# nianticlabs/relpose-gnn

Measured on AMD Instinct MI355X. Metric: graphs/sec (8-node fully-connected, 224x224), higher is better.
Workload: dtype f32; 1 GPU; BASELINE.json configs[1]: batch=32 8-node fully-connected graphs per GPU, 224x224 RGB, fp32, ResNet34 + GNN (D=2048, gnn_recursion=2, droprate=0, eval), random-init weights; nodes_per_graph=8, edges_per_graph=56, streams_per_gpu=2, loaded_library=relpose-gnn_amd/lib/librelpose_gnn_hip.so@88d037e48742

## Files before the change

relpose-gnn_amd/csrc/stem.hip:

```cpp
#include "rpg_common.h"

typedef float f32x16 __attribute__((ext_vector_type(16)));

namespace {

constexpr int ST_NT = 512;
constexpr int PH = 4;
constexpr int CR = 2 * PH + 1;
constexpr int IR = 2 * CR + 5;
constexpr int TWP_MAX = 56;
constexpr int PITCH = 4 * TWP_MAX + 8;
constexpr int KP = 74;
constexpr int NF = 2;
constexpr int NFRAG_MAX = (CR * (2 * TWP_MAX + 1) + 31) / 32;
constexpr int PATCH_FLOATS = 3 * IR * PITCH;
constexpr int POOL_FLOATS = (PH * TWP_MAX + 1) * 64;
constexpr int TAB_DWORDS = NFRAG_MAX * 32 * 4;
constexpr int ST_LDS_BYTES = (PATCH_FLOATS + POOL_FLOATS + TAB_DWORDS) * 4;

struct StemArgs {
    const float* x;
    const float* wpack;
    const float* shift;
    float* out;
    int N, H, W, Hc, Wc, Hp, Wp;
    int TWp, tiles_x, tiles_y, RW, nfrag, total_tiles;
    int nbx, nblk, ncl;
};

__host__ __device__ constexpr int tap_off(int c, int kh, int kw) { return (c * IR + kh) * PITCH + kw; }
__host__ __device__ constexpr int pair_class(int kp) { return kp < 63 ? 0 : (kp < 72 ? 1 : (kp == 72 ? 2 : 0)); }
__host__ __device__ constexpr int pair_off(int kp) {
    return kp < 63 ? tap_off(kp / 21, (kp % 21) / 3, 2 * (kp % 3))
                   : (kp < 72 ? tap_off((kp - 63) / 3, 2 * ((kp - 63) % 3), 6) : (kp == 72 ? tap_off(0, 6, 6) : tap_off(2, 6, 6)));
}

__global__ __launch_bounds__(ST_NT) void stem_pool_kernel(StemArgs a) {
    extern __shared__ __attribute__((aligned(16))) float lds[];
    float* patch = lds;
    unsigned* pooled = reinterpret_cast<unsigned*>(lds + PATCH_FLOATS);
    uint4* tab = reinterpret_cast<uint4*>(lds + PATCH_FLOATS + POOL_FLOATS);
    const int tid = threadIdx.x, lane = tid & 63, h = lane >> 5;
    const int wave = __builtin_amdgcn_readfirstlane(tid >> 6);

    float breg[KP][NF];
#pragma unroll
    for (int kp = 0; kp < KP; ++kp)
#pragma unroll
        for (int nf = 0; nf < NF; ++nf) breg[kp][nf] = a.wpack[(kp * NF + nf) * 64 + lane];
    float sh[NF];
#pragma unroll
    for (int nf = 0; nf < NF; ++nf) sh[nf] = a.shift[32 * nf + (lane & 31)];
    __builtin_amdgcn_s_waitcnt(0x0F70);
#pragma unroll
    for (int kp = 0; kp < KP; ++kp)
#pragma unroll
        for (int nf = 0; nf < NF; ++nf) asm volatile("" : "+v"(breg[kp][nf]));
#pragma unroll
    for (int nf = 0; nf < NF; ++nf) asm volatile("" : "+v"(sh[nf]));
    const unsigned trash = (unsigned)(PH * a.TWp) * 256u;
    const unsigned lane_b = 4u * (unsigned)(lane & 31);
    const int pcol = tid & 255, prow0 = __builtin_amdgcn_readfirstlane(tid >> 8);
    constexpr int NROW = 3 * IR, NPV = (NROW + 1) / 2;
    for (int tile = blockIdx.x; tile < a.total_tiles; tile += gridDim.x) {
        const int n = tile / (a.tiles_y * a.tiles_x);
        const int tr = tile - n * (a.tiles_y * a.tiles_x);
        const int ty = tr / a.tiles_x, tx = tr - ty * a.tiles_x;
        const int P0 = ty * PH, Q0 = tx * a.TWp;
        const int cy0 = 2 * P0 - 1, cx0 = 2 * Q0 - 1;
        const int iy0 = 2 * cy0 - 3, ix0 = 2 * cx0 - 3;
        const int npix = CR * a.RW;
        {
            float pv[NPV];
            {
                const float* img = a.x + (size_t)n * 3 * a.H * a.W;
                const int ix = ix0 + pcol;
                const int ixc = ix < 0 ? 0 : (ix >= a.W ? a.W - 1 : ix);
#pragma unroll
                for (int u = 0; u < NPV; ++u) {
                    int rr = prow0 + 2 * u;
                    rr = rr < NROW ? rr : NROW - 1;
                    const int c = rr / IR, r = rr - c * IR;
                    int iy = iy0 + r;
                    iy = iy < 0 ? 0 : (iy >= a.H ? a.H - 1 : iy);
#ifndef ST_NO_PATCH
                    pv[u] = img[((size_t)c * a.H + iy) * a.W + ixc];
#else
                    pv[u] = 1.f;
#endif
                }
            }
            for (int i = tid; i < (PH * a.TWp + 1) * 16; i += ST_NT) reinterpret_cast<uint4*>(pooled)[i] = make_uint4(0u, 0u, 0u, 0u);
            for (int l = tid; l < (a.nfrag - a.nblk) * 32; l += ST_NT) {
                int ey = CR - 1, ex = l;
                bool in = l < a.RW;
                if (!in && a.ncl > 0) {
                    const int l2 = l - a.RW;
                    ey = l2 / a.ncl;
                    ex = 8 * a.nbx + (l2 - ey * a.ncl);
                    in = ey < CR - 1;
                }
                const int cy = cy0 + ey, cx = cx0 + ex;
                unsigned c4[4] = {trash, trash, trash, trash};
                if (in && (unsigned)cy < (unsigned)a.Hc && (unsigned)cx < (unsigned)a.Wc) {
                    const int r0 = (cy >> 1) - P0, r1 = ((cy + 1) >> 1) - P0, q0 = (cx >> 1) - Q0, q1 = ((cx + 1) >> 1) - Q0;
                    const bool r0v = (unsigned)r0 < (unsigned)PH && P0 + r0 < a.Hp, r1v = r1 != r0 && (unsigned)r1 < (unsigned)PH && P0 + r1 < a.Hp;
                    const bool q0v = (unsigned)q0 < (unsigned)a.TWp && Q0 + q0 < a.Wp, q1v = q1 != q0 && (unsigned)q1 < (unsigned)a.TWp && Q0 + q1 < a.Wp;
                    if (r0v && q0v) c4[0] = (unsigned)(r0 * a.TWp + q0) * 256u;
                    if (r0v && q1v) c4[1] = (unsigned)(r0 * a.TWp + q1) * 256u;
                    if (r1v && q0v) c4[2] = (unsigned)(r1 * a.TWp + q0) * 256u;
                    if (r1v && q1v) c4[3] = (unsigned)(r1 * a.TWp + q1) * 256u;
                }
                tab[l] = make_uint4(c4[0], c4[1], c4[2], c4[3]);
            }
            if (pcol < PITCH) {
                const bool col_ok = pcol < 4 * a.TWp + 7 && (unsigned)(ix0 + pcol) < (unsigned)a.W;
#pragma unroll
                for (int u = 0; u < NPV; ++u) {
                    const int rr = prow0 + 2 * u;
                    const int r = rr - (rr / IR) * IR;
                    const bool ok = col_ok && (unsigned)(iy0 + r) < (unsigned)a.H;
                    if (rr < NROW) patch[rr * PITCH + pcol] = ok ? pv[u] : 0.f;
                }
            }
        }
        __syncthreads();
        for (int f = wave; f < a.nfrag; f += ST_NT / 64) {
            const bool blk = f < a.nblk;
            int oy, ox, by = 0, bx = 0;
            if (blk) {
                by = f / a.nbx; bx = f - by * a.nbx;
                oy = 4 * by + ((lane & 31) >> 3);
                ox = 8 * bx + (lane & 7);
            } else {
                const int l = (f - a.nblk) * 32 + (lane & 31);
                oy = CR - 1; ox = l;
                if (l >= a.RW) {
                    const int l2 = l - a.RW;
                    oy = a.ncl > 0 ? l2 / a.ncl : CR;
                    ox = 8 * a.nbx + (l2 - oy * a.ncl);
                    if (oy >= CR - 1) { oy = 0; ox = 0; }
                }
            }
            const float* q = patch + (2 * oy * PITCH + 2 * ox);
            const float* q0 = q + (h ? 1 : 0);
            const float* q1 = q + (h ? PITCH : 0);
            const float* q2 = q + (h ? IR * PITCH : 0);
            f32x16 acc[NF];
#pragma unroll
            for (int nf = 0; nf < NF; ++nf)
#pragma unroll
                for (int e = 0; e < 16; ++e) acc[nf][e] = 0.f;
#pragma unroll
            for (int kp = 0; kp < KP; ++kp) {
                const int cls = pair_class(kp);
                const float av = (cls == 0 ? q0 : (cls == 1 ? q1 : q2))[pair_off(kp)];
#pragma unroll
                for (int nf = 0; nf < NF; ++nf) {
#ifndef ST_NO_MFMA
                    acc[nf] = __builtin_amdgcn_mfma_f32_32x32x2f32(av, breg[kp][nf], acc[nf], 0, 0, 0);
#else
                    acc[nf][kp & 15] += av * breg[kp][nf];
#endif
                }
            }
#ifdef ST_NO_EPI
            if (a.N == -5)
#endif
            if (blk) {
                const int cyb = cy0 + 4 * by, cxs = cx0 + 8 * bx + 4 * h;
                bool rok[4], cok[4];
#pragma unroll
                for (int t = 0; t < 4; ++t) {
                    rok[t] = (unsigned)(cyb + t) < (unsigned)a.Hc;
                    cok[t] = (unsigned)(cxs + t) < (unsigned)a.Wc;
                }
                const int ra = 2 * by, qa = 4 * bx + 2 * h;
                unsigned cell[3][3];
#pragma unroll
                for (int ri = 0; ri < 3; ++ri)
#pragma unroll
                    for (int qi = 0; qi < 3; ++qi) {
                        const int r = ra - 1 + ri, qq = qa - 1 + qi;
                        const bool ok = (unsigned)r < (unsigned)PH && P0 + r < a.Hp && (unsigned)qq < (unsigned)a.TWp && Q0 + qq < a.Wp;
                        cell[ri][qi] = (ok ? (unsigned)(r * a.TWp + qq) * 256u : trash) + lane_b;
                    }
#pragma unroll
                for (int nf = 0; nf < NF; ++nf) {
                    float c[4][3];
#pragma unroll
                    for (int y = 0; y < 4; ++y) {
                        float v[4];
#pragma unroll
                        for (int xx = 0; xx < 4; ++xx) {
                            const float t = rpg::relu(acc[nf][4 * y + xx] + sh[nf]);
                            v[xx] = rok[y] && cok[xx] ? t : 0.f;
                        }
                        c[y][0] = v[0];
                        c[y][1] = rpg::nan_max3(v[0], v[1], v[2]);
                        c[y][2] = rpg::nan_max(v[2], v[3]);
                    }
#pragma unroll
                    for (int qi = 0; qi < 3; ++qi) {
                        const float m0 = c[0][qi];
                        const float m1 = rpg::nan_max3(c[0][qi], c[1][qi], c[2][qi]);
                        const float m2 = rpg::nan_max(c[2][qi], c[3][qi]);
                        const float m[3] = {m0, m1, m2};
#pragma unroll
                        for (int ri = 0; ri < 3; ++ri) {
                            if ((ri == 0 || qi == 0) && __builtin_amdgcn_ballot_w64(cell[ri][qi] != trash + lane_b) == 0) continue;
#ifndef ST_NO_ATOMICS
                            atomicMax(reinterpret_cast<unsigned*>(reinterpret_cast<char*>(pooled) + cell[ri][qi]) + 32 * nf,
                                      __float_as_uint(m[ri]));
#else
                            asm volatile("" ::"v"(cell[ri][qi]), "v"(m[ri]));
#endif
                        }
                    }
                }
            } else {
                const int l0 = (f - a.nblk) * 32 + 4 * h;
#pragma unroll
                for (int e = 0; e < 16; ++e) {
                    const uint4 cells = tab[l0 + (e & 3) + 8 * (e >> 2)];
                    const unsigned v0 = __float_as_uint(rpg::relu(acc[0][e] + sh[0]));
                    const unsigned v1 = __float_as_uint(rpg::relu(acc[1][e] + sh[1]));
                    const unsigned co[4] = {cells.x, cells.y, cells.z, cells.w};
#pragma unroll
                    for (int k = 0; k < 4; ++k) {
                        if (k > 0 && __builtin_amdgcn_ballot_w64(co[k] != trash) == 0) continue;
                        unsigned* cellp = reinterpret_cast<unsigned*>(reinterpret_cast<char*>(pooled) + (co[k] + lane_b));
#ifndef ST_NO_ATOMICS
                        atomicMax(cellp, v0);
                        atomicMax(cellp + 32, v1);
#else
                        asm volatile("" ::"v"(cellp), "v"(v0), "v"(v1));
#endif
                    }
                }
            }
        }
        __syncthreads();
        for (int i = tid; i < PH * a.TWp * 16; i += ST_NT) {
            const int c4 = i & 15, cell = i >> 4;
            const int r = cell / a.TWp, qq = cell - r * a.TWp;
            const int py = P0 + r, px = Q0 + qq;
            if (py < a.Hp && px < a.Wp)
                reinterpret_cast<uint4*>(a.out)[(((size_t)n * a.Hp + py) * a.Wp + px) * 16 + c4] = reinterpret_cast<const uint4*>(pooled)[i];
        }
        __syncthreads();
    }
}


constexpr int SF_NT = 256, SF_TP = 15, SF_NW = 75;
struct StemSFArgs {
    const float* x;
    const float* wpack;
    const float* shift;
    float* out;
    int N, H, W, Hc, Wc, Hp, Wp;
    int TP, tiles_x, BH, bands;
    unsigned items;
};

__global__ __launch_bounds__(SF_NT) __attribute__((amdgpu_waves_per_eu(2, 2))) void stem_strip_f32_kernel(StemSFArgs a) {
    constexpr int NFH = 1;
    constexpr unsigned SENT = 0x80000000u;
    __shared__ float wl[2 * SF_NW * 64];
    __shared__ __attribute__((aligned(16))) float shl[64];
    const int tid = threadIdx.x, lane = tid & 63, l = lane & 31, h = lane >> 5;
    const int wave = __builtin_amdgcn_readfirstlane(tid >> 6);
    for (int i = tid; i < 2 * SF_NW * 64; i += SF_NT) wl[i] = a.wpack[i];
    if (tid < 64) shl[tid] = a.shift[tid];
    __syncthreads();
    const unsigned b = blockIdx.x, nb = gridDim.x;
    unsigned wg = b;
    if ((nb & 15u) == 0) { const unsigned xcd = b & 7u, k = b >> 3; wg = ((k >> 1) * 8u + xcd) * 2u + (k & 1u); }
    const unsigned item = wg * 4u + (unsigned)wave;
    if (item >= a.items) return;
    const int nf = NFH == 1 ? (int)(item & 1u) : 0;
    unsigned rest = NFH == 1 ? item >> 1 : item;
    const int strip = (int)(rest % (unsigned)a.tiles_x); rest /= (unsigned)a.tiles_x;
    const int band = (int)(rest % (unsigned)a.bands);
    const int n = (int)(rest / (unsigned)a.bands);
    const int Q0 = strip * a.TP, P0 = band * a.BH;
    const int nq = a.TP < a.Wp - Q0 ? a.TP : a.Wp - Q0, np = a.BH < a.Hp - P0 ? a.BH : a.Hp - P0;
    const int H = a.H, W = a.W;
    const bool hi = h != 0;

    const int u = l < 16 ? 2 * l : 2 * (l - 16) + 1;
    int cx = 2 * Q0 - 1 + u;
    cx = cx < 0 ? 0 : (cx >= a.Wc ? a.Wc - 1 : cx);
    unsigned vcol[4];
#pragma unroll
    for (int q = 0; q < 4; ++q) {
        const int col = q < 3 ? 2 * cx - 3 + 2 * q + h : 2 * cx + 3;
        vcol[q] = (unsigned)col < (unsigned)W ? 4u * (unsigned)col : SENT;
    }
    const size_t img_elems = (size_t)3 * H * W;
    const __amdgpu_buffer_rsrc_t rs =
        __builtin_amdgcn_make_buffer_rsrc(const_cast<float*>(a.x) + (size_t)n * img_elems, 0, (unsigned)(img_elems * 4), 0x00020000);

    float win[3][8][4];
#pragma unroll
    for (int c = 0; c < 3; ++c)
#pragma unroll
        for (int sl = 0; sl < 8; ++sl)
#pragma unroll
            for (int q = 0; q < 4; ++q) win[c][sl][q] = 0.f;
    float mx[NFH][16];
    const float* const wl_lane = wl + nf * SF_NW * 64 + lane;
    float* const out_n = a.out + (size_t)n * a.Hp * a.Wp * 64 + 32 * nf + 4 * h;
    auto emit = [&](int py) {
        if (py < P0 || py >= P0 + np) return;
#pragma unroll
        for (int f = 0; f < NFH; ++f) {
            float r[16];
#pragma unroll
            for (int e = 0; e < 16; ++e) {
                const int mi = __builtin_bit_cast(int, mx[f][e]);
                const float right = __builtin_bit_cast(float, __builtin_amdgcn_update_dpp(mi, mi, 0x101, 0xf, 0xf, false));
                const float odd = __builtin_bit_cast(float, __builtin_amdgcn_ds_swizzle(mi, 0x401f));
                r[e] = rpg::nan_max3(mx[f][e], right, odd);
            }
            if (l < nq) {
                float* o = out_n + ((size_t)py * a.Wp + Q0 + l) * 64 + 32 * f;
#pragma unroll
                for (int g = 0; g < 4; ++g) {
                    const float4 sh = *reinterpret_cast<const float4*>(shl + 32 * (nf + f) + 8 * g + 4 * h);
                    float4 v;
                    v.x = rpg::relu(r[4 * g + 0] + sh.x); v.y = rpg::relu(r[4 * g + 1] + sh.y);
                    v.z = rpg::relu(r[4 * g + 2] + sh.z); v.w = rpg::relu(r[4 * g + 3] + sh.w);
                    *reinterpret_cast<float4*>(o + 8 * g) = v;
                }
            }
        }
    };

    const int oy_first = P0 > 0 ? 2 * P0 - 1 : 0;
    int oy_last = 2 * (P0 + np) - 1;
    oy_last = oy_last < a.Hc ? oy_last : a.Hc - 1;
#define RPG_SF_LOAD(SL, ROW)                                                                                                   \
    do {                                                                                                                       \
        const int r_ = (ROW);                                                                                                  \
        if ((unsigned)r_ < (unsigned)H) {                                                                                      \
            _Pragma("unroll") for (int c = 0; c < 3; ++c) {                                                                    \
                const unsigned ro_ = (unsigned)(((c * H + r_) * W) * 4);                                                       \
                _Pragma("unroll") for (int q = 0; q < 4; ++q)                                                                  \
                    win[c][SL][q] = __builtin_bit_cast(float, __builtin_amdgcn_raw_buffer_load_b32(rs, vcol[q] == SENT ? SENT : vcol[q] + ro_, 0, 0)); \
            }                                                                                                                  \
        } else {                                                                                                               \
            _Pragma("unroll") for (int c = 0; c < 3; ++c)                                                                      \
                _Pragma("unroll") for (int q = 0; q < 4; ++q) win[c][SL][q] = 0.f;                                             \
        }                                                                                                                      \
    } while (0)
#define RPG_SF_MFMA(K, B)                                                                                                      \
    do {                                                                                                                       \
        _Pragma("unroll") for (int f = 0; f < NFH; ++f) {                                                                      \
            acc[f] = __builtin_amdgcn_mfma_f32_32x32x2f32(wf[f][(K) % 3], (B), acc[f], 0, 0, 0);                               \
            if ((K) + 2 < SF_NW) wf[f][((K) + 2) % 3] = wl_lane[(f * SF_NW + (K) + 2) * 64];                                   \
            __builtin_amdgcn_sched_barrier(0);                                                                                 \
        }                                                                                                                      \
    } while (0)
#define RPG_SF_ROW(R)                                                                                                          \
    do {                                                                                                                       \
        RPG_SF_LOAD((2 * (R) + 3) & 7, 2 * oy + 3);                                  \
        RPG_SF_LOAD((2 * (R) + 4) & 7, 2 * oy + 4);                                          \
        if (oy >= oy_first) {                                                                                                  \
            f32x16 acc[NFH];         \
            float wf[NFH][3];                                                                                                  \
            _Pragma("unroll") for (int f = 0; f < NFH; ++f) {                                                                  \
                _Pragma("unroll") for (int e = 0; e < 16; ++e) acc[f][e] = 0.f;                                                \
                wf[f][0] = wl_lane[(f * SF_NW + 0) * 64];                                                                      \
                wf[f][1] = wl_lane[(f * SF_NW + 1) * 64];                                                                      \
            }                                                                                                                  \
            __builtin_amdgcn_sched_barrier(0);                                                                                 \
            _Pragma("unroll") for (int kh = 0; kh < 7; ++kh) {                                                                 \
                const int sl_ = (2 * (R) + 5 + kh) & 7, kb_ = 9 * kh + 3 * (kh / 2);                                           \
                _Pragma("unroll") for (int c = 0; c < 3; ++c)                                                                  \
                    _Pragma("unroll") for (int p = 0; p < 3; ++p) RPG_SF_MFMA(kb_ + 3 * c + p, win[c][sl_][p]);                \
                if (kh & 1) {                                                                                                  \
                    _Pragma("unroll") for (int c = 0; c < 3; ++c)                                                              \
                        RPG_SF_MFMA(kb_ + 9 + c, hi ? win[c][sl_][3] : win[c][(sl_ + 7) & 7][3]);                              \
                }                                                                                                              \
                if (kh == 6) {                                                                                                 \
                    _Pragma("unroll") for (int c = 0; c < 3; ++c) RPG_SF_MFMA(kb_ + 9 + c, win[c][sl_][3]);                    \
                }                                                                                                              \
            }                                                                                                                  \
            if (oy == oy_first) {                                                                                              \
                _Pragma("unroll") for (int f = 0; f < NFH; ++f)                                                                \
                    _Pragma("unroll") for (int e = 0; e < 16; ++e) mx[f][e] = acc[f][e];                                    \
            } else {                                                                                                           \
                _Pragma("unroll") for (int f = 0; f < NFH; ++f)                                                                \
                    _Pragma("unroll") for (int e = 0; e < 16; ++e) mx[f][e] = rpg::nan_max(mx[f][e], acc[f][e]);           \
            }                                                                                                                  \
            if ((R) & 1) {                                                                                                     \
                emit((oy - 1) >> 1);                                                                                           \
                _Pragma("unroll") for (int f = 0; f < NFH; ++f)                                                                \
                    _Pragma("unroll") for (int e = 0; e < 16; ++e) mx[f][e] = acc[f][e];                                    \
            }                                                                                                                  \
        }                                                                                                                      \
        ++oy;                                                                                                                  \
    } while (0)

    int oy = (oy_first - 3) & ~3;
    while (oy <= oy_last) {
        RPG_SF_ROW(0);
        if (oy > oy_last) break;
        RPG_SF_ROW(1);
        if (oy > oy_last) break;
        RPG_SF_ROW(2);
        if (oy > oy_last) break;
        RPG_SF_ROW(3);
    }
#undef RPG_SF_ROW
#undef RPG_SF_MFMA
#undef RPG_SF_LOAD
    if (!(oy_last & 1)) emit(oy_last >> 1);
}

}

namespace rpg {

bool stem_pool_supported(int h, int w, int cout) { return tuning().stem.fused && cout == 64 && h >= 1 && w >= 1; }


static int strip_band_rows(long items_per_band, int hp, long slots) {
    int best_bh = hp;
    double best = -1.0;
    for (int bands = 1; bands <= hp; ++bands) {
        const int bh = (hp + bands - 1) / bands;
        if (bh < 7 && bands > 1) break;
        const int nb = (hp + bh - 1) / bh;
        if (nb != bands) continue;
        const long wgs = (items_per_band * nb + 3) / 4;
        const long rounds = (wgs + slots - 1) / slots;
        const double eff = (double)wgs / (double)(rounds * slots) * (2.0 * bh / (2.0 * bh + 2.5)) * ((double)hp / (double)(nb * bh));
        if (eff > best + 1e-9) { best = eff; best_bh = bh; }
    }
    return best_bh;
}

int launch_stem_pool(const float* x_nchw, const float* wpack, const float* shift, float* out, int n, int h, int w,
                     hipStream_t s) {
    if (!x_nchw || !wpack || !shift || !out || n <= 0 || h <= 0 || w <= 0 || !aligned16(out)) return RPG_ERR_BAD_ARG;
    if (tuning().stem.strip && (long)3 * h * w * 4 < (1L << 31)) {
        StemSFArgs sa{};
        sa.x = x_nchw; sa.wpack = wpack + KP * NF * 64; sa.shift = shift; sa.out = out;
        sa.N = n; sa.H = h; sa.W = w;
        sa.Hc = (h + 6 - 7) / 2 + 1; sa.Wc = (w + 6 - 7) / 2 + 1;
        sa.Hp = (sa.Hc + 2 - 3) / 2 + 1; sa.Wp = (sa.Wc + 2 - 3) / 2 + 1;
        sa.tiles_x = (sa.Wp + SF_TP - 1) / SF_TP;
        sa.TP = (sa.Wp + sa.tiles_x - 1) / sa.tiles_x;
        if (tuning().stem.strip_bh > 0) {
            sa.BH = tuning().stem.strip_bh < sa.Hp ? tuning().stem.strip_bh : sa.Hp;
        } else {
            sa.BH = strip_band_rows((long)n * sa.tiles_x * 2, sa.Hp, 2L * num_cus());
        }
        sa.bands = (sa.Hp + sa.BH - 1) / sa.BH;
        const long items = (long)n * sa.bands * sa.tiles_x * 2;
        if (items + 64 < (1L << 32)) {
            sa.items = (unsigned)items;
            const int slot = timing_begin(RPG_TIMER_CONV, s);
            hipLaunchKernelGGL(stem_strip_f32_kernel, dim3((unsigned)((items + 3) / 4)), dim3(SF_NT), 0, s, sa);
            timing_end(slot, 2.0 * (double)n * sa.Hc * sa.Wc * 64.0 * 147.0, s,
                       (double)items * (2.0 * sa.Hp / sa.bands + 1.0) * SF_NW * 4096.0);
            RPG_CHECK_LAUNCH("stem_conv_bn_relu_maxpool (strips)");
            return RPG_OK;
        }
    }
    StemArgs a{};
    a.x = x_nchw; a.wpack = wpack; a.shift = shift; a.out = out;
    a.N = n; a.H = h; a.W = w;
    a.Hc = (h + 6 - 7) / 2 + 1; a.Wc = (w + 6 - 7) / 2 + 1;
    a.Hp = (a.Hc + 2 - 3) / 2 + 1; a.Wp = (a.Wc + 2 - 3) / 2 + 1;
    a.tiles_x = (a.Wp + TWP_MAX - 1) / TWP_MAX;
    a.TWp = (a.Wp + a.tiles_x - 1) / a.tiles_x;
    a.tiles_y = (a.Hp + PH - 1) / PH;
    a.RW = 2 * a.TWp + 1;
    a.nbx = a.RW / 8;
    a.nblk = 2 * a.nbx;
    a.ncl = a.RW - 8 * a.nbx;
    a.nfrag = a.nblk + (a.RW + 8 * a.ncl + 31) / 32;
    const long total = (long)n * a.tiles_y * a.tiles_x;
    if (total >= (1L << 31) || (long)n * 3 * h * w >= (1L << 40)) return RPG_ERR_BAD_ARG;
    a.total_tiles = (int)total;
    int dev = 0;
    if (hipGetDevice(&dev) != hipSuccess || dev < 0 || dev >= 64) dev = 0;
    static bool attr[64] = {};
    if (!attr[dev]) {
        (void)hipFuncSetAttribute(reinterpret_cast<const void*>(stem_pool_kernel), hipFuncAttributeMaxDynamicSharedMemorySize,
                                  ST_LDS_BYTES);
        attr[dev] = true;
    }
    const int slot = timing_begin(RPG_TIMER_CONV, s);
    const int grid = (int)(total < num_cus() ? total : num_cus());
    hipLaunchKernelGGL(stem_pool_kernel, dim3(grid), dim3(ST_NT), ST_LDS_BYTES, s, a);
    timing_end(slot, 2.0 * (double)n * a.Hc * a.Wc * 64.0 * 147.0, s, (double)total * a.nfrag * KP * NF * 4096.0);
    RPG_CHECK_LAUNCH("stem_conv_bn_relu_maxpool");
    return RPG_OK;
}

}

extern "C" int rpg_stem_conv7x7s2_bn_relu_maxpool_f32(const float* x_nchw, const float* wpack, const float* shift,
                                                      float* y_nhwc, int n, int h, int w, void* stream) {
    return rpg::launch_stem_pool(x_nchw, wpack, shift, y_nhwc, n, h, w, rpg::as_stream(stream));
}

extern "C" int rpg_stem_pair_table(int* tap_a , int* tap_b ) {
    if (!tap_a || !tap_b) return RPG_ERR_BAD_ARG;
    for (int kp = 0; kp < KP; ++kp) {
        const int off = pair_off(kp);
        const int c = off / (IR * PITCH), kh = (off / PITCH) % IR, kw = off % PITCH;
        tap_a[3 * kp] = c; tap_a[3 * kp + 1] = kh; tap_a[3 * kp + 2] = kw;
        const int cls = pair_class(kp);
        int cb = c + (cls == 2), khb = kh + (cls == 1), kwb = kw + (cls == 0);
        if (cb > 2 || khb > 6 || kwb > 6) cb = -1;
        tap_b[3 * kp] = cb; tap_b[3 * kp + 1] = khb; tap_b[3 * kp + 2] = kwb;
    }
    return RPG_OK;
}
```

relpose-gnn_amd/csrc/tuning.h:

```cpp
#pragma once
#include "../../include/relpose_gnn_hip.h"

namespace rpg {

struct Tuning {
    struct Gemm {
        int force_tile;
        int bk;
        int epi_lds, streamk;
        int fast;
        int waves8;
        int sk_min_its;
        int fold_k;
        int lin112;
        int inkernel_fixup;
        int fixup_prio;
    } gemm;
    struct Gnn {
        int split, fuse_agg;
        int mean_first;
    } gnn;
    struct Wino {
        int on;
        int min_blocks;
        int split;
        int split_steps;
        int persist;
        int combine_max;
        int wino2d;
    } wino;
    struct Bf16 {
        int bk, fast, tile, dma, linear_dma, lean_epi, pair, persist, tail;
        int patch, stages;
        int chunk, chunk_mb;
        int fuse_block;
        int ws64;
        int fused_stem;
        int stem_strip;
        int stem_strip_bh;
    } bf16;
    struct Stem {
        int fused;
        int strip, strip_bh;
    } stem;
};

struct TuningRow {
    int key;
    const char* name;
    int def;
    bool (*valid)(int);
    void (*decode)(Tuning&, int);
};

constexpr int kTuningKeys = 32;

#define RPG_TUNING_ROW(NAME, def, valid, decode) \
    {RPG_TUNE_##NAME, #NAME, def, [](int v) -> bool { (void)v; return valid; }, [](Tuning& t, int v) { (void)t; (void)v; decode; }}

inline constexpr TuningRow kTuningRows[kTuningKeys] = {
    RPG_TUNING_ROW(TILE, -1, true, t.gemm.force_tile = v),
    RPG_TUNING_ROW(BK, 0, v == 0 || v == 16 || v == 32, t.gemm.bk = v),
    RPG_TUNING_ROW(EPILOGUE, 1, true, t.gemm.epi_lds = v != 0),
    RPG_TUNING_ROW(STREAMK, 1, true, t.gemm.streamk = v != 0),
    RPG_TUNING_ROW(WINOGRAD, 1, v >= 0 && !(v > 3 && v < 16),
                   if (v >= 16) { t.wino.on = 1; t.wino.min_blocks = v; } else { t.wino.on = v; t.wino.min_blocks = 16; }),
    RPG_TUNING_ROW(GNN_SPLIT, 1, true, t.gnn.split = v != 0),
    RPG_TUNING_ROW(BF16_BK, 32, v == 32 || v == 64, t.bf16.bk = v),
    RPG_TUNING_ROW(FAST_LOADER, 1, true, t.gemm.fast = v != 0),
    RPG_TUNING_ROW(WINO_SPLIT, 1, v >= 0 && v <= 96,
                   t.wino.split = v != 0; t.wino.split_steps = v >= 2 ? v : 3),
    RPG_TUNING_ROW(BF16_FAST, 1, true, t.bf16.fast = v != 0),
    RPG_TUNING_ROW(FUSED_STEM, 1, true,
                   t.stem.fused = (v & 1) != 0; t.stem.strip = (v & 128) != 0; t.stem.strip_bh = (v >> 8) > 0 ? (v >> 8) : 0;
                   t.bf16.fused_stem = (v & 1) != 0; t.bf16.stem_strip = (v & 2) ? 0 : ((v & 32) ? 1 : 9);
                   t.bf16.stem_strip_bh = (v >> 8) > 0 ? (v >> 8) : 0),
    RPG_TUNING_ROW(WAVES8, 1, true, t.gemm.waves8 = v != 0),
    RPG_TUNING_ROW(WINO_SHORT, 0, v >= 0, ),
    RPG_TUNING_ROW(GNN_FUSE_AGG, 1, true,
                   t.gnn.fuse_agg = v != 0; t.gnn.mean_first = v != 0 && v != 2),
    RPG_TUNING_ROW(WINO_PERSIST, 1, v >= 0 && v <= 2, t.wino.persist = v),
    RPG_TUNING_ROW(BF16_TILE, -1, v >= -1 && v <= 3, t.bf16.tile = v),
    RPG_TUNING_ROW(BF16_DMA, 1, v >= 0 && v <= 40, t.bf16.dma = v),
    RPG_TUNING_ROW(BF16_PATCH, 1, v >= 0 && v % 10 <= 4 && v <= 14,
                   t.bf16.stages = v >= 10 ? 3 : 4; t.bf16.patch = v % 10),
#ifdef RPG_PROBE_WS64
    RPG_TUNING_ROW(BF16_WS64, 0, v >= 0 && v <= 2, t.bf16.ws64 = v),
#else
    RPG_TUNING_ROW(BF16_WS64, 0, v == 0, t.bf16.ws64 = v),
#endif
    RPG_TUNING_ROW(SK_MIN_ITS, 8, v >= 1 && v <= 4096, t.gemm.sk_min_its = v),
    RPG_TUNING_ROW(INKERNEL_FIXUP, 0, v >= 0 && v <= 7,
                   t.gemm.inkernel_fixup = v & 3; t.wino.combine_max = (v & 4) ? 32 : 8),
    RPG_TUNING_ROW(BF16_CHUNK, 0, v >= 0,
                   t.bf16.chunk = v & 4095; t.bf16.chunk_mb = (v >> 12) ? (v >> 12) : 64),
#ifdef RPG_PROBE_WINO2D
    RPG_TUNING_ROW(WINO2D, 0, v >= 0 && v <= 2, t.wino.wino2d = v),
#else
    RPG_TUNING_ROW(WINO2D, 0, v == 0, t.wino.wino2d = v),
#endif
    RPG_TUNING_ROW(BF16_LEAN_EPI, 1, true, t.bf16.lean_epi = v != 0),
    RPG_TUNING_ROW(BF16_LINEAR_DMA, 0, v == 0 || (v >= 10 && v <= 19), t.bf16.linear_dma = v),
    RPG_TUNING_ROW(BF16_PERSIST, 0, true, t.bf16.persist = v != 0),
    RPG_TUNING_ROW(FOLD_K, 256, v >= 0 && v % 64 == 0, t.gemm.fold_k = v),
    RPG_TUNING_ROW(BF16_FUSE_BLOCK, 3, true, t.bf16.fuse_block = v & 7),
    RPG_TUNING_ROW(BF16_TAIL, 1, v >= 0 && v <= 7, t.bf16.tail = v & 7),
    RPG_TUNING_ROW(LIN112, 3, v >= 0 && v <= 3, t.gemm.lin112 = v),
    RPG_TUNING_ROW(FIXUP_PRIO, 0, true, t.gemm.fixup_prio = v != 0),
    RPG_TUNING_ROW(BF16_PAIR, 1, true, t.bf16.pair = v != 0),
};
#undef RPG_TUNING_ROW

constexpr bool tuning_rows_in_key_order() {
    for (int k = 0; k < kTuningKeys; ++k)
        if (kTuningRows[k].key != k) return false;
    return true;
}
static_assert(tuning_rows_in_key_order(), "kTuningRows[k] must be the row of key k");

struct TuningState {
    int raw[kTuningKeys];
    Tuning decoded;
};

constexpr TuningState default_tuning_state() {
    TuningState s{};
    for (int k = 0; k < kTuningKeys; ++k) {
        s.raw[k] = kTuningRows[k].def;
        kTuningRows[k].decode(s.decoded, s.raw[k]);
    }
    return s;
}

inline TuningState g_tuning_state = default_tuning_state();

inline const Tuning& tuning() { return g_tuning_state.decoded; }

inline const TuningRow* tuning_row(int key) { return key >= 0 && key < kTuningKeys ? &kTuningRows[key] : nullptr; }

inline int set_tuning(int key, int value) {
    const TuningRow* row = tuning_row(key);
    if (!row || !row->valid(value)) return RPG_ERR_BAD_ARG;
    g_tuning_state.raw[key] = value;
    row->decode(g_tuning_state.decoded, value);
    return RPG_OK;
}

inline int get_tuning(int key, int* value, int* default_value) {
    const TuningRow* row = tuning_row(key);
    if (!row) return RPG_ERR_BAD_ARG;
    if (value) *value = g_tuning_state.raw[key];
    if (default_value) *default_value = row->def;
    return RPG_OK;
}

}
```

Before: 3186 graphs/s.

## Add exact-strip fp32 stem conv+pool kernel and make it the default path

Adds a new strip kernel for the fused 7x7 stem conv + BN + ReLU + maxpool. Each wave keeps a sliding register window of input rows loaded through buffer loads, with out-of-range rows and columns masked via a sentinel offset. It runs one chain of MFMA 32x32x2 f32 over the exact filter taps per conv row, with weights staged in LDS. With default tuning (strip bit off, tile bit off), this kernel now replaces the previous tiled stem path. The goal is to cut redundant input staging and LDS traffic in the stem, at the cost of more register pressure and extra per-lane gather loads.

Result: no change. 3212 graphs/s (median of 6 runs) (+0.8%).

```diff
diff --git a/relpose-gnn_amd/csrc/stem.hip b/relpose-gnn_amd/csrc/stem.hip
--- a/relpose-gnn_amd/csrc/stem.hip
+++ b/relpose-gnn_amd/csrc/stem.hip
@@ -420,6 +420,166 @@
     if (!(oy_last & 1)) emit(oy_last >> 1);
 }
 
+__device__ __forceinline__ float pick(bool second, float b, float a) { return second ? b : a; }
+
+__global__ __launch_bounds__(SF_NT) __attribute__((amdgpu_waves_per_eu(2, 2))) void stem_strip_exact_kernel(StemSFArgs a) {
+    constexpr unsigned SENT = 0x80000000u;
+    __shared__ float wl[KP * NF * 64];
+    __shared__ __attribute__((aligned(16))) float shl[64];
+    const int tid = threadIdx.x, lane = tid & 63, l = lane & 31, h = lane >> 5;
+    const int wave = __builtin_amdgcn_readfirstlane(tid >> 6);
+    for (int i = tid; i < KP * NF * 64; i += SF_NT) wl[i] = a.wpack[i];
+    if (tid < 64) shl[tid] = a.shift[tid];
+    __syncthreads();
+    const unsigned b = blockIdx.x, nb = gridDim.x;
+    unsigned wg = b;
+    if ((nb & 15u) == 0) { const unsigned xcd = b & 7u, k = b >> 3; wg = ((k >> 1) * 8u + xcd) * 2u + (k & 1u); }
+    const unsigned item = wg * 4u + (unsigned)wave;
+    if (item >= a.items) return;
+    const int nf = (int)(item & 1u);
+    unsigned rest = item >> 1;
+    const int strip = (int)(rest % (unsigned)a.tiles_x); rest /= (unsigned)a.tiles_x;
+    const int band = (int)(rest % (unsigned)a.bands);
+    const int n = (int)(rest / (unsigned)a.bands);
+    const int Q0 = strip * a.TP, P0 = band * a.BH;
+    const int nq = a.TP < a.Wp - Q0 ? a.TP : a.Wp - Q0, np = a.BH < a.Hp - P0 ? a.BH : a.Hp - P0;
+    const int H = a.H, W = a.W;
+    const bool hi = h != 0;
+
+    const int u = l < 16 ? 2 * l : 2 * (l - 16) + 1;
+    int cx = 2 * Q0 - 1 + u;
+    cx = cx < 0 ? 0 : (cx >= a.Wc ? a.Wc - 1 : cx);
+    unsigned vcol[5];
+#pragma unroll
+    for (int q = 0; q < 5; ++q) {
+        const int col = q < 3 ? 2 * cx - 3 + 2 * q + h : (q == 3 ? 2 * cx + 3 : 2 * cx + 3 + h);
+        vcol[q] = (unsigned)col < (unsigned)W ? 4u * (unsigned)col : SENT;
+    }
+    const size_t img_elems = (size_t)3 * H * W;
+    const __amdgpu_buffer_rsrc_t rs =
+        __builtin_amdgcn_make_buffer_rsrc(const_cast<float*>(a.x) + (size_t)n * img_elems, 0, (unsigned)(img_elems * 4), 0x00020000);
+
+    float win[3][8][4];
+#pragma unroll
+    for (int c = 0; c < 3; ++c)
+#pragma unroll
+        for (int sl = 0; sl < 8; ++sl)
+#pragma unroll
+            for (int q = 0; q < 4; ++q) win[c][sl][q] = 0.f;
+    float mx[16];
+    const float* const wl_lane = wl + nf * 64 + lane;
+    float* const out_n = a.out + (size_t)n * a.Hp * a.Wp * 64 + 32 * nf + 4 * h;
+    auto emit = [&](int py) {
+        if (py < P0 || py >= P0 + np) return;
+        float r[16];
+#pragma unroll
+        for (int e = 0; e < 16; ++e) {
+            const int mi = __builtin_bit_cast(int, mx[e]);
+            const float right = __builtin_bit_cast(float, __builtin_amdgcn_update_dpp(mi, mi, 0x101, 0xf, 0xf, false));
+            const float odd = __builtin_bit_cast(float, __builtin_amdgcn_ds_swizzle(mi, 0x401f));
+            r[e] = rpg::nan_max3(mx[e], right, odd);
+        }
+        if (l < nq) {
+            float* o = out_n + ((size_t)py * a.Wp + Q0 + l) * 64;
+#pragma unroll
+            for (int g = 0; g < 4; ++g) {
+                const float4 sh = *reinterpret_cast<const float4*>(shl + 32 * nf + 8 * g + 4 * h);
+                float4 v;
+                v.x = rpg::relu(r[4 * g + 0] + sh.x); v.y = rpg::relu(r[4 * g + 1] + sh.y);
+                v.z = rpg::relu(r[4 * g + 2] + sh.z); v.w = rpg::relu(r[4 * g + 3] + sh.w);
+                *reinterpret_cast<float4*>(o + 8 * g) = v;
+            }
+        }
+    };
+
+    const int oy_first = P0 > 0 ? 2 * P0 - 1 : 0;
+    int oy_last = 2 * (P0 + np) - 1;
+    oy_last = oy_last < a.Hc ? oy_last : a.Hc - 1;
+    const int row_min = 2 * oy_first - 3 > 0 ? 2 * oy_first - 3 : 0;
+    const unsigned row_cnt = (unsigned)(H - row_min);
+#define RPG_SX_SLOT(R, KH) ((2 * (R) + 5 + (KH)) & 7)
+#define RPG_SX_LOAD(C, SL, ROW, EVEN)                                                                                          \
+    do {                                                                                                                       \
+        const int r_ = (ROW);                                                                                                  \
+        const bool rok_ = (unsigned)(r_ - row_min) < row_cnt;        \
+        unsigned ro_ = (unsigned)((((C) * H + r_) * W) * 4);                                                                   \
+        asm volatile("" : "+s"(ro_));         \
+        _Pragma("unroll") for (int q = 0; q < 4; ++q) {                                                                        \
+            const unsigned vc_ = vcol[(q == 3 && (C) == 2 && (EVEN)) ? 4 : q];                                                 \
+            win[C][SL][q] = __builtin_bit_cast(float, __builtin_amdgcn_raw_buffer_load_b32(rs, rok_ && vc_ != SENT ? vc_ + ro_ : SENT, 0, 0)); \
+        }                                                                                                                      \
+    } while (0)
+#define RPG_SX_MFMA(K, B)                                                                                                      \
+    do {                                                                                                                       \
+        acc = __builtin_amdgcn_mfma_f32_32x32x2f32(wf[(K) % 3], (B), acc, 0, 0, 0);                                            \
+        if ((K) + 2 < KP) wf[((K) + 2) % 3] = wl_lane[((K) + 2) * (NF * 64)];                                                  \
+        __builtin_amdgcn_sched_barrier(0);                                                                                     \
+    } while (0)
+#define RPG_SX_CHAIN(R)                                                                                                        \
+    do {                                                                                                                       \
+        f32x16 acc;                                                                                                            \
+        float wf[3], va0[3];                                                                                                   \
+        _Pragma("unroll") for (int e = 0; e < 16; ++e) acc[e] = 0.f;                                                           \
+        wf[0] = wl_lane[0];                                                                                                    \
+        wf[1] = wl_lane[NF * 64];                                                                                              \
+        _Pragma("unroll") for (int c = 0; c < 3; ++c)                                                                          \
+            va0[c] = pick(hi, win[c][RPG_SX_SLOT(R, 1)][3], win[c][RPG_SX_SLOT(R, 0)][3]);                                     \
+        __builtin_amdgcn_sched_barrier(0);                                                                                     \
+        _Pragma("unroll") for (int c = 0; c < 3; ++c) {                                                                        \
+            _Pragma("unroll") for (int kh = 0; kh < 7; ++kh) {                                                                 \
+                _Pragma("unroll") for (int p = 0; p < 3; ++p)                                                                  \
+                    RPG_SX_MFMA(21 * c + 3 * kh + p, win[c][RPG_SX_SLOT(R, kh)][p]);                                           \
+                if (kh == 0) RPG_SX_LOAD(c, RPG_SX_SLOT(R, 8), 2 * oy + 5, true);            \
+            }                                                                                                                  \
+        }                                                                                                                      \
+        _Pragma("unroll") for (int c = 0; c < 3; ++c) {                                                                        \
+            RPG_SX_MFMA(63 + 3 * c, va0[c]);                                                                                   \
+            _Pragma("unroll") for (int j = 1; j < 3; ++j)                                                                      \
+                RPG_SX_MFMA(63 + 3 * c + j, pick(hi, win[c][RPG_SX_SLOT(R, 2 * j + 1)][3], win[c][RPG_SX_SLOT(R, 2 * j)][3])); \
+        }                                                                                                                      \
+        RPG_SX_MFMA(72, pick(hi, win[1][RPG_SX_SLOT(R, 6)][3], win[0][RPG_SX_SLOT(R, 6)][3]));                                 \
+        RPG_SX_MFMA(73, win[2][RPG_SX_SLOT(R, 6)][3]);                                                                         \
+        if (oy == oy_first) {                                                                                                  \
+            _Pragma("unroll") for (int e = 0; e < 16; ++e) mx[e] = acc[e];                                                     \
+        } else {                                                                                                               \
+            _Pragma("unroll") for (int e = 0; e < 16; ++e) mx[e] = rpg::nan_max(mx[e], acc[e]);                                \
+        }                                                                                                                      \
+        if (oy & 1) {                                                                                                          \
+            emit((oy - 1) >> 1);                                                                                               \
+            _Pragma("unroll") for (int e = 0; e < 16; ++e) mx[e] = acc[e];                                                     \
+        }                                                                                                                      \
+    } while (0)
+#define RPG_SX_ROW(R)                                                                                                          \
+    do {                                                                                                                       \
+        if (oy < oy_first) {                 \
+            _Pragma("unroll") for (int c = 0; c < 3; ++c) RPG_SX_LOAD(c, RPG_SX_SLOT(R, 7), 2 * oy + 4, false);                \
+            _Pragma("unroll") for (int c = 0; c < 3; ++c) RPG_SX_LOAD(c, RPG_SX_SLOT(R, 8), 2 * oy + 5, true);                 \
+        } else {                                                                                                               \
+            _Pragma("unroll") for (int c = 0; c < 3; ++c) RPG_SX_LOAD(c, RPG_SX_SLOT(R, 7), 2 * oy + 4, false);                \
+            RPG_SX_CHAIN(R);                                   \
+        }                                                                                                                      \
+        ++oy;                                                                                                                  \
+    } while (0)
+
+    int oy = (oy_first - 4) & ~3;
+    while (oy <= oy_last) {
+        RPG_SX_ROW(0);
+        if (oy > oy_last) break;
+        RPG_SX_ROW(1);
+        if (oy > oy_last) break;
+        RPG_SX_ROW(2);
+        if (oy > oy_last) break;
+        RPG_SX_ROW(3);
+    }
+#undef RPG_SX_ROW
+#undef RPG_SX_CHAIN
+#undef RPG_SX_MFMA
+#undef RPG_SX_LOAD
+#undef RPG_SX_SLOT
+    if (!(oy_last & 1)) emit(oy_last >> 1);
+}
+
+
 }
 
 namespace rpg {
@@ -446,9 +606,11 @@
 int launch_stem_pool(const float* x_nchw, const float* wpack, const float* shift, float* out, int n, int h, int w,
                      hipStream_t s) {
     if (!x_nchw || !wpack || !shift || !out || n <= 0 || h <= 0 || w <= 0 || !aligned16(out)) return RPG_ERR_BAD_ARG;
-    if (tuning().stem.strip && (long)3 * h * w * 4 < (1L << 31)) {
+    const bool old_strips = tuning().stem.strip != 0;
+    if ((old_strips || !tuning().stem.tile) && (long)3 * h * w * 4 < (1L << 31)) {
         StemSFArgs sa{};
-        sa.x = x_nchw; sa.wpack = wpack + KP * NF * 64; sa.shift = shift; sa.out = out;
+        sa.x = x_nchw; sa.shift = shift; sa.out = out;
+        sa.wpack = old_strips ? wpack + KP * NF * 64 : wpack;
         sa.N = n; sa.H = h; sa.W = w;
         sa.Hc = (h + 6 - 7) / 2 + 1; sa.Wc = (w + 6 - 7) / 2 + 1;
         sa.Hp = (sa.Hc + 2 - 3) / 2 + 1; sa.Wp = (sa.Wc + 2 - 3) / 2 + 1;
@@ -464,10 +626,24 @@
         if (items + 64 < (1L << 32)) {
             sa.items = (unsigned)items;
             const int slot = timing_begin(RPG_TIMER_CONV, s);
-            hipLaunchKernelGGL(stem_strip_f32_kernel, dim3((unsigned)((items + 3) / 4)), dim3(SF_NT), 0, s, sa);
+            const dim3 grid((unsigned)((items + 3) / 4));
+            if (old_strips) {
+                hipLaunchKernelGGL(stem_strip_f32_kernel, grid, dim3(SF_NT), 0, s, sa);
+                timing_end(slot, 2.0 * (double)n * sa.Hc * sa.Wc * 64.0 * 147.0, s,
+                           (double)items * (2.0 * sa.Hp / sa.bands + 1.0) * SF_NW * 4096.0);
+                RPG_CHECK_LAUNCH("stem_conv_bn_relu_maxpool (strips)");
+                return RPG_OK;
+            }
+            hipLaunchKernelGGL(stem_strip_exact_kernel, grid, dim3(SF_NT), 0, s, sa);
+            long rows = 0;
+            for (int bd = 0; bd < sa.bands; ++bd) {
+                const int p0 = bd * sa.BH, p1 = p0 + sa.BH < sa.Hp ? p0 + sa.BH : sa.Hp;
+                const int first = p0 > 0 ? 2 * p0 - 1 : 0, last = 2 * p1 - 1 < sa.Hc ? 2 * p1 - 1 : sa.Hc - 1;
+                rows += last - first + 1;
+            }
             timing_end(slot, 2.0 * (double)n * sa.Hc * sa.Wc * 64.0 * 147.0, s,
-                       (double)items * (2.0 * sa.Hp / sa.bands + 1.0) * SF_NW * 4096.0);
-            RPG_CHECK_LAUNCH("stem_conv_bn_relu_maxpool (strips)");
+                       (double)n * sa.tiles_x * 2.0 * (double)rows * KP * 4096.0);
+            RPG_CHECK_LAUNCH("stem_conv_bn_relu_maxpool (exact strips)");
             return RPG_OK;
         }
     }
diff --git a/relpose-gnn_amd/csrc/tuning.h b/relpose-gnn_amd/csrc/tuning.h
--- a/relpose-gnn_amd/csrc/tuning.h
+++ b/relpose-gnn_amd/csrc/tuning.h
@@ -42,6 +42,7 @@
     struct Stem {
         int fused;
         int strip, strip_bh;
+        int tile;
     } stem;
 };
 
@@ -73,6 +74,7 @@
     RPG_TUNING_ROW(BF16_FAST, 1, true, t.bf16.fast = v != 0),
     RPG_TUNING_ROW(FUSED_STEM, 1, true,
                    t.stem.fused = (v & 1) != 0; t.stem.strip = (v & 128) != 0; t.stem.strip_bh = (v >> 8) > 0 ? (v >> 8) : 0;
+                   t.stem.tile = (v & 2) != 0;
                    t.bf16.fused_stem = (v & 1) != 0; t.bf16.stem_strip = (v & 2) ? 0 : ((v & 32) ? 1 : 9);
                    t.bf16.stem_strip_bh = (v >> 8) > 0 ? (v >> 8) : 0),
     RPG_TUNING_ROW(WAVES8, 1, true, t.gemm.waves8 = v != 0),
```
